# ssttuu/go-pbrt

Hardware: AMD Instinct MI355X
Metric: Mpaths/s (samples×pixels/s) at 1920×1080, 64 spp; 1/2/4/8-GPU scaling + HBM GB/s vs roofline (higher is better)
Workload: dtype f64

## Files before the change

### go-pbrt_amd/csrc/k_chain.h

```cpp
#pragma once
#pragma clang fp contract(off)

#include "render_common.h"

namespace pbrtk {

template <bool kX>
__device__ __forceinline__ uint32_t ring_d(const Cursor& c, const SpecSampler& ss, uint32_t d) {
    if (!kX || c.rri < 0 || d == kBadExactD || c.rrn == 0) return d;
    return kRrFlag | (d == kBadSpecD ? kRrTailBad : d);
}

__device__ __forceinline__ int uni(int v) { return __builtin_amdgcn_readfirstlane(v); }
__device__ __forceinline__ uint32_t uni(uint32_t v) { return (uint32_t)__builtin_amdgcn_readfirstlane((int)v); }
__device__ __forceinline__ float uni(float v) { return __int_as_float(__builtin_amdgcn_readfirstlane(__float_as_int(v))); }
__device__ __forceinline__ uint64_t uni(uint64_t v) {
    return (uint64_t)uni((uint32_t)(v >> 32)) << 32 | uni((uint32_t)v);
}
__device__ __forceinline__ int64_t uni(int64_t v) { return (int64_t)uni((uint64_t)v); }
__device__ __forceinline__ CiGroup uni(const CiGroup& s) {
    CiGroup u;
    u.S = uni(s.S);
    u.pi = uni(s.pi);
    u.npx = uni(s.npx);
    u.A = uni(s.A);
    u.head = uni(s.head);
    u.nxt = uni(s.nxt);
    u.kh = uni(s.kh);
    u.phase = uni(s.phase);
    u.reissue = uni(s.reissue);
    u.rb0 = uni(s.rb0);
    u.rb1 = uni(s.rb1);
    u.nb = uni(s.nb);
    u.nnx = uni(s.nnx);
    u.nps = uni(s.nps);
    u.dcnt = uni(s.dcnt);
    u.dsum = uni(s.dsum);
    u.dsq = uni(s.dsq);
    return u;
}

template <int kW, int kDepth, bool kX, int kEu, bool kSpWin, bool kMulti>
__global__ __launch_bounds__(kWave * kW) __attribute__((amdgpu_waves_per_eu(kEu > 0 ? kEu : kDepth < 0 ? PBRT_CI_MESH_EU_WAVES : kX ? PBRT_CI_X_EU_WAVES : PBRT_CI_EU_WAVES, 8))) void k_chain_ci(
    DevScene sc, RenderParams rp, ChainLayout lay, const PcgJump* __restrict__ jump, WaveBufs wb, int64_t slot_base,
    int64_t nslots_batch, int lanes_per_tile, int ring_size, Counters* __restrict__ ctr,
    const uint32_t* __restrict__ order, uint32_t* __restrict__ ticks, int cstride, uint32_t* __restrict__ prog) {
    extern __shared__ __attribute__((aligned(16))) unsigned char lds[];
    const uint64_t t_begin = wall_clock64();
    if (prog && threadIdx.x == 0) __hip_atomic_fetch_add(&prog[0], 1u, __ATOMIC_RELAXED, __HIP_MEMORY_SCOPE_AGENT);
    const uint32_t cs = cstride == 1 ? 1u : 2u;
    constexpr int kT = kWave * kW;
    __shared__ uint16_t stack_lds[kDepth > 0 ? kDepth * kT : 1];
#ifdef PBRT_CI_DENSE_WALK
    __shared__ __attribute__((aligned(16))) unsigned char dense_lds[kDepth > 0 ? 16 : kW * kDenseScratch];
#endif
    __shared__ CiGroup gs[kCiMaxGroups];
    __shared__ uint64_t sh_state;
    __shared__ uint32_t sh_draws;
    __shared__ int sh_act;
    __shared__ int wcnt[kW];
#ifdef PBRT_CI_DIAG
    __shared__ uint32_t dh[64];
#endif
    static_assert(!kMulti || kW == 1, "several tiles per wave: one-wave workgroups only");
    const int tid = threadIdx.x, lane = tid & (kWave - 1), wv = kW > 1 ? uni(tid / kWave) : 0;
    stage_nodes(sc);
    const int L = kMulti ? lanes_per_tile : kT, G = kMulti ? kWave / L : 1;
    const int g = kMulti ? lane / L : 0, gl = kMulti ? lane - g * L : tid;
    const int64_t blk = order ? (int64_t)order[blockIdx.x] : (int64_t)blockIdx.x;
    const uint32_t R = (uint32_t)ring_size;
    const PcgJump& J = *jump;
    double* s1d = lay.s1d >= 0 ? (double*)(lds + lay.s1d) : nullptr;
    uint16_t* other = (uint16_t*)(lds + lay.other);
    uint32_t* vbuf = (uint32_t*)(lds + lay.vbuf);
    constexpr bool kNps = kW > 1 && !kX;
    const bool nps_on = kNps && rp.ci_nps != 0 && cstride == 1;
    constexpr uint32_t kNpsMinStats = 16;
    constexpr bool kStats = !kX && (kW > 1 || kDepth < 0);
    const float zcap = nps_on ? 3.0f : rp.ci_scap >= 0 ? 0.1f * (float)rp.ci_scap : kDepth < 0 ? 1.5f : 0.0f;
    auto ring_of = [&](int64_t pix) -> RingEnt* {
        return (RingEnt*)(lds + lay.ring) + (size_t)(nps_on ? (int)(pix & 1) : g) * R;
    };
    auto rpar = [&](int64_t pix) -> int { return nps_on ? (int)(pix & 1) : 0; };
    ChainCache* pcs = (ChainCache*)(lds + lay.pcs);
    uint16_t* stack = stack_lds + tid;
    const int n = rp.spp, ndims = rp.ndims;
#ifndef PBRT_CI_TAILCAP
#define PBRT_CI_TAILCAP 1
#endif
    const uint32_t dmax = (uint32_t)(camera_draws(ndims) + 8 * (rp.max_depth + 1) + 8);
    const pbrt_camera_desc& cam = *sc.camera;
    const unsigned long long gmask = !kMulti || L >= 64 ? ~0ULL : (((1ULL << (L & 63)) - 1ULL) << (g * L));
    const int64_t bs = blk * G + g;
    const uint64_t inc = pcg_inc_of((uint64_t)tile_of_slot(rp, slot_base + (bs < nslots_batch ? bs : 0)));
#ifdef PBRT_CI_DIAG
    unsigned long long steps = 0, busy = 0;
    unsigned long long ph[8] = {0, 0, 0, 0, 0, 0, 0, 0};
    long long tprev = clock64();
    auto mark = [&](int k) {
        long long now = clock64();
        ph[k] += (unsigned long long)(now - tprev);
        tprev = now;
    };
    if (tid < 64) dh[tid] = 0;
#define CI_DIAG(x) x
#else
    auto mark = [](int) {};
#define CI_DIAG(x)
#endif
    if (tid < G) {
        const int64_t b = blk * G + tid;
        CiGroup& s = gs[tid];
        s.pi = 0;
        s.kh = 1;
        s.A = s.head = s.nxt = 0;
        s.rb0 = s.rb1 = 0;
        s.nb = s.nnx = 0;
        s.nps = 0;
        s.dcnt = 0;
        s.dsum = s.dsq = 0.0f;
        s.reissue = 0;
        if (b < nslots_batch) {
            int64_t x0, y0, x1, y1;
            tile_bounds(rp, tile_of_slot(rp, slot_base + b), x0, y0, x1, y1);
            Pcg seed;
            pcg_seed(seed, (uint64_t)tile_of_slot(rp, slot_base + b));
            s.S = seed.state;
            s.npx = (x1 - x0) * (y1 - y0);
            s.phase = s.npx > 0 ? 0 : 2;
            wb.tile_npx[b] = 0;
        } else {
            s.S = 0;
            s.npx = 0;
            s.phase = 2;
        }
    }
    __syncthreads();

    uint32_t cancel_poll = 0;
    uint64_t last_host_poll = t_begin;
    uint32_t off = kNoOff;
    int opi_r = -1;
#ifdef PBRT_CI_LDS_STATE
    constexpr bool kLdsState = true;
#else
    constexpr bool kLdsState = kX;
#endif
    __shared__ Spec xs_beta[kLdsState ? kT : 1];
    __shared__ double xs_eta[kLdsState ? kT : 1];
    constexpr bool kStIssue = !kMulti;
    __shared__ uint64_t xs_st0[kLdsState && !kStIssue ? kT : 1];
    uint64_t st0_r = 0;
    Spec beta_r = spec(1);
    double eta_r = 1.0;
    uint64_t& st0 = [&]() -> uint64_t& { if constexpr (kLdsState && !kStIssue) return xs_st0[tid]; else return st0_r; }();
    Spec& beta = [&]() -> Spec& { if constexpr (kLdsState) return xs_beta[tid]; else return beta_r; }();
    double& eta_scale = [&]() -> double& { if constexpr (kLdsState) return xs_eta[tid]; else return eta_r; }();
    st0 = 0;
    beta = spec(1);
    eta_scale = 1.0;
    bool tracing = false;
    Cursor c;
    c.rri = -1;
    c.rrn = 0;
    c.rng.state = 0;
    c.rng.inc = inc;
    c.draws = 0;
    c.cur1d = c.cur2d = 0;
    c.k = -1;
    c.kdep = 0;
    int bounces = 1;
    Ray ray;
    ray.o = ray.d = V3{0, 0, 0};
    ray.tmax = kInf;
    ray.time = 0;

    for (;;) {
        for (int q = 0; q < G; q++) {
            while (gs[q].phase == 0) {
                const int64_t bq = blk * G + q;
                const int64_t tile = tile_of_slot(rp, slot_base + bq);
                const uint64_t incq = pcg_inc_of((uint64_t)tile);
                const int64_t pi = gs[q].pi;
                const int64_t rec = bq * wb.ppt + pi;
                int64_t x0, y0, x1, y1;
                tile_bounds(rp, tile, x0, y0, x1, y1);
                const int64_t px = x0 + pi % (x1 - x0), py = y0 + pi / (x1 - x0);
                double* gs1d = wb.s1d + rec * wb.s1d_stride;
                double* sp = s1d ? s1d : gs1d;
                const uint64_t S1 = start_pixel_wave<kSpWin>(rp, J, gs[q].S, incq, sp, other, vbuf, &sh_state, &sh_draws);
                if (s1d)
                    for (int idx = tid; idx < ndims * n; idx += kT) gs1d[idx] = s1d[idx];
                const double time_u = sp[1 < n ? 1 : 0];
                __syncthreads();
                const bool spec_ran = nps_on && gs[q].nps != 0;
                if (!spec_ran) {
                    RingEnt* rq = nps_on ? ring_of(pi) : (RingEnt*)(lds + lay.ring) + (size_t)q * R;
                    for (uint32_t i = (uint32_t)tid; i < R; i += kT) rq[i].tag = kNoOff;
                }
                PixelRec& pr = wb.prec[rec];
                const int hit0 = pr.hit, panic0 = pr.panic0;
                if (tid == 0) {
                    if (prog)
                        __hip_atomic_fetch_add(&prog[2], 1u, __ATOMIC_RELAXED, __HIP_MEMORY_SCOPE_AGENT);
                    const uint64_t now = wall_clock64();
                    const bool host = now - last_host_poll >= 100000;
                    if (host) last_host_poll = now;
                    if (cancel_requested(sc, host))
                        for (int q2 = 0; q2 < G; q2++) gs[q2].phase = 2;
                }
                if (tid == 0 && gs[q].phase == 0) {
                    if (hit0)
                        pr.si.time = camera_ray(cam, (double)px, (double)py, time_u, V2{0.0, 0.0}).time;
                    ChainCache& pq = pcs[2 * q + rpar(pi)];
                    pq.si = pr.si;
                    pq.b = pr.b;
                    if constexpr (kX) pq.x = pr.x;
                    pq.wo = pr.wo;
                    pq.hit = hit0;
                    CiGroup& s = gs[q];
                    s.S = S1;
                    s.A += sh_draws;
                    s.head = s.A;
                    s.nxt = (spec_ran && s.A >= s.nb) ? max(s.nnx, s.A) : s.A;
                    if (!spec_ran) {
                        if (rpar(pi)) s.rb1 = s.A;
                        else s.rb0 = s.A;
                    }
                    s.nps = 0;
                    s.kh = 1;
                    s.reissue = 0;
                    wb.tile_npx[bq] = (int32_t)(pi + 1);
                    if (panic0) {
                        s.phase = 2;
                    } else if (hit0) {
                        s.phase = 1;
                    } else {
                        if (ndims < 2) {
                            s.S = pcg_advance(J, S1, incq, (uint64_t)(n - 1) * camera_draws(ndims));
                            s.A += (uint32_t)(n - 1) * camera_draws(ndims);
                        }
                        s.pi = pi + 1;
                        s.phase = s.pi < s.npx ? 0 : 2;
                    }
                }
                __syncthreads();
            }
        }
        mark(0);
        bool any_chain = false;
        for (int q = 0; q < G; q++) any_chain |= gs[q].phase == 1;
        if (!any_chain) break;
        CI_DIAG(steps++;)

        CiGroup sg;
        if constexpr (kMulti) sg = gs[g];
        else sg = uni(gs[0]);
        const int64_t rec = bs * wb.ppt + sg.pi;
        const SpecSampler ss{wb.s1d + rec * wb.s1d_stride, n, ndims,
                             kX && wb.rrb ? wb.rrb + bs * kCiMaxRing : nullptr};
        {
            const bool idle = sg.phase == 1 && off == kNoOff;
            const unsigned long long m = __ballot(idle) & gmask;
            int nidle = __popcll(m);
            int rank;
            if constexpr (kMulti) rank = __popcll(m & ((1ULL << lane) - 1ULL));
            else rank = (int)__builtin_amdgcn_mbcnt_hi((uint32_t)(m >> 32), __builtin_amdgcn_mbcnt_lo((uint32_t)m, 0u));
            if (kW > 1) {
                if (lane == 0) wcnt[wv] = nidle;
                __syncthreads();
                int before = 0, tot = 0;
                for (int w = 0; w < kW; w++) {
                    const int cw = wcnt[w];
                    before += w < wv ? cw : 0;
                    tot += cw;
                }
                rank += before;
                nidle = tot;
            }
            const int re = (sg.reissue && nidle > 0) ? 1 : 0;
            const uint32_t nx0 = sg.nxt;
            const int avail = nx0 < sg.head + R ? (int)((sg.head + R - nx0 + cs - 1) / cs) : 0;
#if PBRT_CI_TAILCAP
            const uint32_t tail = sg.head + (uint32_t)(n - 1 - sg.kh) * dmax;
            const int capn = nx0 <= tail ? (int)((tail - nx0) / cs) + 1 : 0;
            int nspec = min(min(nidle - re, avail), capn);
            if (kStats && zcap > 0.0f && sg.dcnt >= kNpsMinStats) {
                const float rem = (float)(n - 1 - sg.kh);
                const float mu = sg.dsum / (float)sg.dcnt;
                const float sd = sqrtf(fmaxf(0.0f, sg.dsq / (float)sg.dcnt - mu * mu));
                const uint32_t scap = sg.head + (uint32_t)(rem * mu + zcap * sd * sqrtf(rem));
                nspec = min(nspec, nx0 <= scap ? (int)((scap - nx0) / cs) + 1 : 0);
            }
#else
            const int nspec = min(nidle - re, avail);
#endif
            int nspec1 = 0;
            if (kNps && sg.phase == 1 && sg.nps) {
                const int avail1 = sg.nnx < sg.nb + R ? (int)(sg.nb + R - sg.nnx) : 0;
                nspec1 = max(0, min(nidle - re - max(nspec, 0), avail1));
            }
            uint32_t o = kNoOff;
            bool exact = false;
            int opix = (int)sg.pi;
            if (idle) {
                if (re && rank == 0) {
                    o = sg.head;
                    exact = true;
                } else {
                    rank -= re;
                    if (rank < nspec) {
                        o = nx0 + cs * (uint32_t)rank;
                    } else if (kNps && rank - nspec < nspec1) {
                        o = sg.nnx + (uint32_t)(rank - nspec);
                        opix = (int)sg.pi + 1;
                    }
                }
            }
            if (gl == 0 && sg.phase == 1) {
                gs[g].nxt = nx0 + cs * (uint32_t)max(nspec, 0);
                if (kNps) gs[g].nnx = sg.nnx + (uint32_t)nspec1;
                CI_DIAG(ph[5] += (unsigned long long)(max(nspec, 0) + nspec1 + re);)
                CI_DIAG(ph[7] += (unsigned long long)nspec1;)
                if (re) gs[g].reissue = 0;
            }
            if (o != kNoOff) {
                off = o;
                if (kNps) opi_r = opix;
                RingEnt& e = ring_of(opix)[(off - (rpar(opix) ? sg.rb1 : sg.rb0)) & (R - 1u)];
                if constexpr (kStIssue) {
                    const uint64_t st = pcg_advance(J, sg.S, inc, (uint64_t)(o - sg.A));
                    e.st = st;
                    c.rng.state = st;
                } else {
                    st0 = pcg_advance(J, sg.S, inc, (uint64_t)(o - sg.A));
                    c.rng.state = st0;
                }
                c.draws = 0;
                c_camera(c, ndims);
                c.k = exact ? sg.kh : -1;
                c.kdep = 0;
                if constexpr (kX) {
                    c.rri = (!exact && ss.rrb) ? (int)((off - sg.rb0) & (R - 1u)) : -1;
                    c.rrn = 0;
                }
                beta = spec(1);
                eta_scale = 1.0;
                bounces = 1;
                const ChainCache& pc = pcs[2 * g + rpar(opix)];
                const int r = traj_scatter<kX>(sc, pc.si, pc.b, pc.x, pc.wo, c, ss, beta, eta_scale, bounces, ray,
                                               rp.max_depth, rp.rr_threshold);
                tracing = r == 0;
                if (r != 0) {
                    if constexpr (!kStIssue) e.st = st0;
                    e.d = ring_d<kX>(c, ss, r == 1 ? c.draws : (c.k >= 0 ? kBadExactD : kBadSpecD));
                    e.tag = off;
                    off = kNoOff;
                }
            }
        }
        const int64_t opi = kNps ? (int64_t)opi_r : sg.pi;
        mark(1);
        CI_DIAG(const unsigned long long tbusy = __ballot(tracing); if (lane == 0) busy += (unsigned long long)__popcll(tbusy);)
#ifdef PBRT_CI_DENSE_WALK
        const bool dense = kDepth == 0 && sc.dense_ok && sc.use_lds_nodes;
        int panic = 0, best = -1;
        V3 ph{0, 0, 0};
        if (dense) bvh_walk_dense(sc, ray, tracing, panic, best, ph, dense_lds + (size_t)wv * kDenseScratch);
        if (tracing) {
            if (!dense) bvh_walk<false, kT, PBRT_CHAIN_LB, (kDepth < 0)>(sc, ray, stack, panic, best, ph);
#else
        if (tracing) {
            int panic = 0, best;
            V3 ph;
            bvh_walk<false, kT, PBRT_CHAIN_LB, (kDepth < 0)>(sc, ray, stack, panic, best, ph);
#endif
            mark(2);
            uint32_t d = kNoOff;
            if (panic) {
                d = c.k >= 0 ? kBadExactD : kBadSpecD;
            } else if (best < 0) {
                d = c.draws;
            } else {
                SI si;
                prim_si(sc, best, ray, ph, si);
                BSDF b;
                BSDFX x;
                if ((kX ? compute_bsdf_x(sc, si, b, x) : compute_bsdf(sc, si, b)) < 0) {
                    d = c.k >= 0 ? kBadExactD : kBadSpecD;
                } else {
                    const int r = traj_scatter<kX>(sc, si, b, x, ray.d, c, ss, beta, eta_scale, bounces, ray,
                                                   rp.max_depth, rp.rr_threshold);
                    if (r == 1) d = c.draws;
                    else if (r == 2) d = c.k >= 0 ? kBadExactD : kBadSpecD;
                }
            }
            if (d != kNoOff) {
                RingEnt& e = ring_of(opi)[(off - (rpar(opi) ? sg.rb1 : sg.rb0)) & (R - 1u)];
                if constexpr (!kStIssue) e.st = st0;
                e.d = ring_d<kX>(c, ss, d);
                e.tag = off;
                off = kNoOff;
                tracing = false;
            }
        }
        mark(3);
        __syncthreads();
        if (gl == 0 && sg.phase == 1) {
            CiGroup s = gs[g];
            if ((++cancel_poll & 127u) == 0) {
                const uint64_t now = wall_clock64();
                const bool host = now - last_host_poll >= 100000;
                if (host) last_host_poll = now;
                if (cancel_requested(sc, host)) s.phase = 2;
            }
            RingEnt* rcur = ring_of(s.pi);
            const uint32_t rbase = rpar(s.pi) ? s.rb1 : s.rb0;
            for (; s.phase == 1;) {
                RingEnt& e = rcur[(s.head - rbase) & (R - 1u)];
                if (e.tag != s.head) break;
                uint32_t d = e.d;
                if (kX && d < kBadExactD && (d & kRrFlag)) {
                    const RrBranches& b = ss.rrb[(s.head - rbase) & (R - 1u)];
                    d = (d & kRrTailBad) == kRrTailBad ? kBadSpecD : (d & kRrTailBad);
                    for (uint32_t i = 0; i < b.n; i++) {
                        const uint32_t cd = b.cd[i];
                        if (ss.s1d[(int)(cd & 0xFFu) * n + s.kh] < b.q[i]) {
                            d = cd >> 8;
                            break;
                        }
                    }
                }
                if (d == kBadSpecD) {
                    e.tag = kNoOff;
                    s.reissue = 1;
                    break;
                }
                wb.memb[rec * n + s.kh] = e.st;
                if (d == kBadExactD) {
                    wb.prec[rec].nvalid = s.kh + 1;
                    s.phase = 2;
                    break;
                }
                CI_DIAG(atomicAdd(&dh[min(d / 2u, 63u)], 1u);)
                CI_DIAG(if (d > dmax) ph[6]++;)
                CI_DIAG(if (d & 1u) atomicAdd(&ctr->odd_d, 1ull);)
                if (kStats) {
                    s.dcnt++;
                    s.dsum += (float)d;
                    s.dsq += (float)d * (float)d;
                }
                s.kh++;
                s.head += d;
                if (s.kh >= n) {
                    s.S = pcg_advance(J, s.S, inc, (uint64_t)(s.head - s.A));
                    s.A = s.head;
                    s.pi++;
                    s.phase = s.pi < s.npx ? 0 : 2;
                    break;
                }
            }
            if (s.nxt < s.head || (cs == 2u && ((s.nxt ^ s.head) & 1u))) s.nxt = s.head;
            int act = 0;
            const int left = n - s.kh;
            const bool stats = s.dcnt >= kNpsMinStats;
            if (nps_on && s.phase == 1 && !s.nps && (left == 1 || (stats && left <= rp.ci_nps)) &&
                s.pi + 1 < s.npx) {
                const PixelRec& pn = wb.prec[rec + 1];
                if (pn.hit && !pn.panic0) {
                    float lo = 0.0f;
                    if (left > 1) {
                        const float mu = s.dsum / (float)s.dcnt;
                        const float sd = sqrtf(fmaxf(0.0f, s.dsq / (float)s.dcnt - mu * mu));
                        lo = fmaxf(0.0f, (float)left * mu - 3.0f * sd * sqrtf((float)left));
                    }
                    s.nps = 1;
                    s.nb = s.head + (uint32_t)lo + (uint32_t)rp.sp_events;
                    s.nnx = s.nb;
                    if (rpar(s.pi + 1)) s.rb1 = s.nb;
                    else s.rb0 = s.nb;
                    act = 1;
                }
            }
            if (kNps) sh_act = act;
            CiGroup& gw = gs[g];
            gw.S = s.S;
            gw.A = s.A;
            gw.pi = s.pi;
            gw.head = s.head;
            gw.nxt = s.nxt;
            gw.kh = s.kh;
            gw.phase = s.phase;
            gw.reissue = s.reissue;
            if (kStats) {
                gw.dcnt = s.dcnt;
                gw.dsum = s.dsum;
                gw.dsq = s.dsq;
            }
            if (kNps) {
                gw.nps = s.nps;
                gw.nb = s.nb;
                gw.nnx = s.nnx;
                gw.rb0 = s.rb0;
                gw.rb1 = s.rb1;
            }
        }
        if (kNps && tid == 0 && !(gl == 0 && sg.phase == 1)) sh_act = 0;
        __syncthreads();
        if (kNps && sh_act) {
            const CiGroup s3 = uni(gs[0]);
            RingEnt* rn = ring_of(s3.pi + 1);
            for (uint32_t i = (uint32_t)tid; i < R; i += kT) rn[i].tag = kNoOff;
            if (tid == 0) {
                const PixelRec& pn = wb.prec[rec + 1];
                ChainCache& pc = pcs[2 * g + rpar(s3.pi + 1)];
                pc.si = pn.si;
                pc.b = pn.b;
                pc.wo = pn.wo;
                pc.hit = pn.hit;
            }
        }
        if (off != kNoOff) {
            const CiGroup s2 = gs[g];
            bool keep = false;
            if ((!kNps || opi == s2.pi) && s2.phase == 1)
                keep = !(off < s2.head || (cs == 2u && ((off ^ s2.head) & 1u)) ||
                         (PBRT_CI_TAILCAP && off > s2.head + (uint32_t)(n - 1 - s2.kh) * dmax));
            else if (kNps && opi == s2.pi && s2.phase == 0)
                keep = s2.nps != 0;
            else if (kNps && opi == s2.pi + 1 && s2.phase == 1)
                keep = s2.nps != 0;
            if (!keep) {
                off = kNoOff;
                tracing = false;
            }
        }
        mark(4);
    }
#ifdef PBRT_CI_DIAG
    __syncthreads();
    if (tid < 64 && dh[tid]) atomicAdd(&ctr->dhist[tid], (unsigned long long)dh[tid]);
    if (tid == 0) {
        atomicAdd(&ctr->windows, steps);
        for (int k = 0; k < 8; k++) atomicAdd(&ctr->phase[k], ph[k]);
        atomicAdd(&ctr->nps_issued, ph[7]);
    }
    if (lane == 0) atomicAdd(&ctr->busy, busy);
#endif
#undef CI_DIAG
    if (prog) {
        __threadfence();
        __syncthreads();
    }
    if (tid == 0) {
        if (prog && G == 1 && bs < nslots_batch) {
            const uint32_t pos = __hip_atomic_fetch_add(&prog[1], 1u, __ATOMIC_RELAXED, __HIP_MEMORY_SCOPE_AGENT);
            __hip_atomic_store(&prog[kProgHead + pos], (uint32_t)bs, __ATOMIC_RELEASE, __HIP_MEMORY_SCOPE_AGENT);
        }
        if (ticks && G == 1 && bs < nslots_batch) {
            const uint64_t t_end = wall_clock64();
            ticks[bs] = (uint32_t)min(t_end - t_begin, (uint64_t)0xFFFFFFFFu);
#ifdef PBRT_CI_DIAG
            ticks[nslots_batch + bs] = (uint32_t)t_begin;
            ticks[2 * nslots_batch + bs] = (uint32_t)t_end;
#endif
        }
    }
}

}
```

Measured before the change: 371.2.

## Reorder chain loop so fresh and hit scatters share one traj_scatter call site

Restructures the chain-issue loop into traverse, scatter and walk_drop lambdas. For depth-limited, non-window kernels it rotates the loop so traversal and ring drain run at the top of the iteration, and a single scatter call handles both freshly issued chains and BVH hits. This removes the duplicated traj_scatter call site, which is meant to cut code size, register pressure and divergent execution of two scatter paths. The rotation changes the order of phases relative to the barriers and hoists sg, rec and ss out of the loop, which risks subtle state-ordering bugs.

```diff
diff --git a/go-pbrt_amd/csrc/k_chain.h b/go-pbrt_amd/csrc/k_chain.h
--- a/go-pbrt_amd/csrc/k_chain.h
+++ b/go-pbrt_amd/csrc/k_chain.h
@@ -95,11 +95,11 @@
     const uint64_t inc = pcg_inc_of((uint64_t)tile_of_slot(rp, slot_base + (bs < nslots_batch ? bs : 0)));
 #ifdef PBRT_CI_DIAG
     unsigned long long steps = 0, busy = 0;
-    unsigned long long ph[8] = {0, 0, 0, 0, 0, 0, 0, 0};
+    unsigned long long ph_cyc[8] = {0, 0, 0, 0, 0, 0, 0, 0};
     long long tprev = clock64();
     auto mark = [&](int k) {
         long long now = clock64();
-        ph[k] += (unsigned long long)(now - tprev);
+        ph_cyc[k] += (unsigned long long)(now - tprev);
         tprev = now;
     };
     if (tid < 64) dh[tid] = 0;
@@ -175,7 +175,216 @@
     ray.tmax = kInf;
     ray.time = 0;
 
+    CiGroup sg;
+    if constexpr (kMulti) sg = gs[g];
+    else sg = uni(gs[0]);
+    int64_t rec = bs * wb.ppt + sg.pi;
+    SpecSampler ss{wb.s1d + rec * wb.s1d_stride, n, ndims, kX && wb.rrb ? wb.rrb + bs * kCiMaxRing : nullptr};
+
+    constexpr bool kOneScatter = kDepth >= 0 && !kSpWin;
+    using Both = std::integral_constant<int, 0>;
+    using Fresh = std::integral_constant<int, 1>;
+    using Hits = std::integral_constant<int, 2>;
+    int best = -1;
+    V3 ph{0, 0, 0};
+    auto traverse = [&]() __attribute__((always_inline)) {
+        const int64_t opi = kNps ? (int64_t)opi_r : sg.pi;
+        best = -1;
+        int panic = 0;
+#ifdef PBRT_CI_DENSE_WALK
+        const bool dense = kDepth == 0 && sc.dense_ok && sc.use_lds_nodes;
+        if (dense) bvh_walk_dense(sc, ray, tracing, panic, best, ph, dense_lds + (size_t)wv * kDenseScratch);
+        if (tracing) {
+            if (!dense) bvh_walk<false, kT, PBRT_CHAIN_LB, (kDepth < 0)>(sc, ray, stack, panic, best, ph);
+#else
+        if (tracing) {
+            bvh_walk<false, kT, PBRT_CHAIN_LB, (kDepth < 0)>(sc, ray, stack, panic, best, ph);
+#endif
+            if (panic || best < 0) {
+                RingEnt& e = ring_of(opi)[(off - (rpar(opi) ? sg.rb1 : sg.rb0)) & (R - 1u)];
+                if constexpr (!kStIssue) e.st = st0;
+                e.d = ring_d<kX>(c, ss, panic ? (c.k >= 0 ? kBadExactD : kBadSpecD) : c.draws);
+                e.tag = off;
+                off = kNoOff;
+                tracing = false;
+            }
+        }
+    };
+    auto scatter = [&](auto which, bool fresh) __attribute__((always_inline)) {
+        constexpr int kWhich = decltype(which)::value;
+        const bool first = kWhich == Fresh::value ? true : kWhich == Hits::value ? false : fresh;
+        if (kWhich == Fresh::value ? fresh : kWhich == Hits::value ? tracing : (fresh || tracing)) {
+            const int64_t spi = kNps ? (int64_t)opi_r : sg.pi;
+            SI si;
+            BSDF b;
+            BSDFX x;
+            V3 wo = ray.d;
+            bool ok = true;
+            if (first) {
+                const ChainCache& pc = pcs[2 * g + rpar(spi)];
+                si = pc.si;
+                b = pc.b;
+                if constexpr (kX) x = pc.x;
+                wo = pc.wo;
+            } else {
+                prim_si(sc, best, ray, ph, si);
+                ok = (kX ? compute_bsdf_x(sc, si, b, x) : compute_bsdf(sc, si, b)) >= 0;
+            }
+            const int r = !ok ? 2
+                              : traj_scatter<kX>(sc, si, b, x, wo, c, ss, beta, eta_scale, bounces, ray, rp.max_depth,
+                                                 rp.rr_threshold);
+            tracing = r == 0;
+            if (r != 0) {
+                RingEnt& e = ring_of(spi)[(off - (rpar(spi) ? sg.rb1 : sg.rb0)) & (R - 1u)];
+                if constexpr (!kStIssue) e.st = st0;
+                e.d = ring_d<kX>(c, ss, r == 1 ? c.draws : (c.k >= 0 ? kBadExactD : kBadSpecD));
+                e.tag = off;
+                off = kNoOff;
+            }
+        }
+    };
+    auto walk_drop = [&]() __attribute__((always_inline)) {
+        const int64_t opi = kNps ? (int64_t)opi_r : sg.pi;
+        __syncthreads();
+        if (gl == 0 && sg.phase == 1) {
+            CiGroup s = gs[g];
+            if ((++cancel_poll & 127u) == 0) {
+                const uint64_t now = wall_clock64();
+                const bool host = now - last_host_poll >= 100000;
+                if (host) last_host_poll = now;
+                if (cancel_requested(sc, host)) s.phase = 2;
+            }
+            RingEnt* rcur = ring_of(s.pi);
+            const uint32_t rbase = rpar(s.pi) ? s.rb1 : s.rb0;
+            for (; s.phase == 1;) {
+                RingEnt& e = rcur[(s.head - rbase) & (R - 1u)];
+                if (e.tag != s.head) break;
+                uint32_t d = e.d;
+                if (kX && d < kBadExactD && (d & kRrFlag)) {
+                    const RrBranches& b = ss.rrb[(s.head - rbase) & (R - 1u)];
+                    d = (d & kRrTailBad) == kRrTailBad ? kBadSpecD : (d & kRrTailBad);
+                    for (uint32_t i = 0; i < b.n; i++) {
+                        const uint32_t cd = b.cd[i];
+                        if (ss.s1d[(int)(cd & 0xFFu) * n + s.kh] < b.q[i]) {
+                            d = cd >> 8;
+                            break;
+                        }
+                    }
+                }
+                if (d == kBadSpecD) {
+                    e.tag = kNoOff;
+                    s.reissue = 1;
+                    break;
+                }
+                wb.memb[rec * n + s.kh] = e.st;
+                if (d == kBadExactD) {
+                    wb.prec[rec].nvalid = s.kh + 1;
+                    s.phase = 2;
+                    break;
+                }
+                CI_DIAG(atomicAdd(&dh[min(d / 2u, 63u)], 1u);)
+                CI_DIAG(if (d > dmax) ph_cyc[6]++;)
+                CI_DIAG(if (d & 1u) atomicAdd(&ctr->odd_d, 1ull);)
+                if (kStats) {
+                    s.dcnt++;
+                    s.dsum += (float)d;
+                    s.dsq += (float)d * (float)d;
+                }
+                s.kh++;
+                s.head += d;
+                if (s.kh >= n) {
+                    s.S = pcg_advance(J, s.S, inc, (uint64_t)(s.head - s.A));
+                    s.A = s.head;
+                    s.pi++;
+                    s.phase = s.pi < s.npx ? 0 : 2;
+                    break;
+                }
+            }
+            if (s.nxt < s.head || (cs == 2u && ((s.nxt ^ s.head) & 1u))) s.nxt = s.head;
+            int act = 0;
+            const int left = n - s.kh;
+            const bool stats = s.dcnt >= kNpsMinStats;
+            if (nps_on && s.phase == 1 && !s.nps && (left == 1 || (stats && left <= rp.ci_nps)) &&
+                s.pi + 1 < s.npx) {
+                const PixelRec& pn = wb.prec[rec + 1];
+                if (pn.hit && !pn.panic0) {
+                    float lo = 0.0f;
+                    if (left > 1) {
+                        const float mu = s.dsum / (float)s.dcnt;
+                        const float sd = sqrtf(fmaxf(0.0f, s.dsq / (float)s.dcnt - mu * mu));
+                        lo = fmaxf(0.0f, (float)left * mu - 3.0f * sd * sqrtf((float)left));
+                    }
+                    s.nps = 1;
+                    s.nb = s.head + (uint32_t)lo + (uint32_t)rp.sp_events;
+                    s.nnx = s.nb;
+                    if (rpar(s.pi + 1)) s.rb1 = s.nb;
+                    else s.rb0 = s.nb;
+                    act = 1;
+                }
+            }
+            if (kNps) sh_act = act;
+            CiGroup& gw = gs[g];
+            gw.S = s.S;
+            gw.A = s.A;
+            gw.pi = s.pi;
+            gw.head = s.head;
+            gw.nxt = s.nxt;
+            gw.kh = s.kh;
+            gw.phase = s.phase;
+            gw.reissue = s.reissue;
+            if (kStats) {
+                gw.dcnt = s.dcnt;
+                gw.dsum = s.dsum;
+                gw.dsq = s.dsq;
+            }
+            if (kNps) {
+                gw.nps = s.nps;
+                gw.nb = s.nb;
+                gw.nnx = s.nnx;
+                gw.rb0 = s.rb0;
+                gw.rb1 = s.rb1;
+            }
+        }
+        if (kNps && tid == 0 && !(gl == 0 && sg.phase == 1)) sh_act = 0;
+        __syncthreads();
+        if (kNps && sh_act) {
+            const CiGroup s3 = uni(gs[0]);
+            RingEnt* rn = ring_of(s3.pi + 1);
+            for (uint32_t i = (uint32_t)tid; i < R; i += kT) rn[i].tag = kNoOff;
+            if (tid == 0) {
+                const PixelRec& pn = wb.prec[rec + 1];
+                ChainCache& pc = pcs[2 * g + rpar(s3.pi + 1)];
+                pc.si = pn.si;
+                pc.b = pn.b;
+                pc.wo = pn.wo;
+                pc.hit = pn.hit;
+            }
+        }
+        if (off != kNoOff) {
+            const CiGroup s2 = gs[g];
+            bool keep = false;
+            if ((!kNps || opi == s2.pi) && s2.phase == 1)
+                keep = !(off < s2.head || (cs == 2u && ((off ^ s2.head) & 1u)) ||
+                         (PBRT_CI_TAILCAP && off > s2.head + (uint32_t)(n - 1 - s2.kh) * dmax));
+            else if (kNps && opi == s2.pi && s2.phase == 0)
+                keep = s2.nps != 0;
+            else if (kNps && opi == s2.pi + 1 && s2.phase == 1)
+                keep = s2.nps != 0;
+            if (!keep) {
+                off = kNoOff;
+                tracing = false;
+            }
+        }
+    };
+
     for (;;) {
+        if constexpr (kOneScatter) {
+            CI_DIAG(const unsigned long long tbusy = __ballot(tracing); if (lane == 0) busy += (unsigned long long)__popcll(tbusy);)
+            traverse();
+            mark(2);
+            walk_drop();
+            mark(4);
+        }
         for (int q = 0; q < G; q++) {
             while (gs[q].phase == 0) {
                 const int64_t bq = blk * G + q;
@@ -188,7 +397,8 @@
                 const int64_t px = x0 + pi % (x1 - x0), py = y0 + pi / (x1 - x0);
                 double* gs1d = wb.s1d + rec * wb.s1d_stride;
                 double* sp = s1d ? s1d : gs1d;
-                const uint64_t S1 = start_pixel_wave<kSpWin>(rp, J, gs[q].S, incq, sp, other, vbuf, &sh_state, &sh_draws);
+                uint64_t S1;
+                [[clang::always_inline]] S1 = start_pixel_wave<kSpWin>(rp, J, gs[q].S, incq, sp, other, vbuf, &sh_state, &sh_draws);
                 if (s1d)
                     for (int idx = tid; idx < ndims * n; idx += kT) gs1d[idx] = s1d[idx];
                 const double time_u = sp[1 < n ? 1 : 0];
@@ -253,12 +463,11 @@
         if (!any_chain) break;
         CI_DIAG(steps++;)
 
-        CiGroup sg;
         if constexpr (kMulti) sg = gs[g];
         else sg = uni(gs[0]);
-        const int64_t rec = bs * wb.ppt + sg.pi;
-        const SpecSampler ss{wb.s1d + rec * wb.s1d_stride, n, ndims,
-                             kX && wb.rrb ? wb.rrb + bs * kCiMaxRing : nullptr};
+        rec = bs * wb.ppt + sg.pi;
+        ss.s1d = wb.s1d + rec * wb.s1d_stride;
+        bool fresh = false;
         {
             const bool idle = sg.phase == 1 && off == kNoOff;
             const unsigned long long m = __ballot(idle) & gmask;
@@ -320,8 +529,8 @@
             if (gl == 0 && sg.phase == 1) {
                 gs[g].nxt = nx0 + cs * (uint32_t)max(nspec, 0);
                 if (kNps) gs[g].nnx = sg.nnx + (uint32_t)nspec1;
-                CI_DIAG(ph[5] += (unsigned long long)(max(nspec, 0) + nspec1 + re);)
-                CI_DIAG(ph[7] += (unsigned long long)nspec1;)
+                CI_DIAG(ph_cyc[5] += (unsigned long long)(max(nspec, 0) + nspec1 + re);)
+                CI_DIAG(ph_cyc[7] += (unsigned long long)nspec1;)
                 if (re) gs[g].reissue = 0;
             }
             if (o != kNoOff) {
@@ -347,203 +556,32 @@
                 beta = spec(1);
                 eta_scale = 1.0;
                 bounces = 1;
-                const ChainCache& pc = pcs[2 * g + rpar(opix)];
-                const int r = traj_scatter<kX>(sc, pc.si, pc.b, pc.x, pc.wo, c, ss, beta, eta_scale, bounces, ray,
-                                               rp.max_depth, rp.rr_threshold);
-                tracing = r == 0;
-                if (r != 0) {
-                    if constexpr (!kStIssue) e.st = st0;
-                    e.d = ring_d<kX>(c, ss, r == 1 ? c.draws : (c.k >= 0 ? kBadExactD : kBadSpecD));
-                    e.tag = off;
-                    off = kNoOff;
-                }
-            }
-        }
-        const int64_t opi = kNps ? (int64_t)opi_r : sg.pi;
-        mark(1);
-        CI_DIAG(const unsigned long long tbusy = __ballot(tracing); if (lane == 0) busy += (unsigned long long)__popcll(tbusy);)
-#ifdef PBRT_CI_DENSE_WALK
-        const bool dense = kDepth == 0 && sc.dense_ok && sc.use_lds_nodes;
-        int panic = 0, best = -1;
-        V3 ph{0, 0, 0};
-        if (dense) bvh_walk_dense(sc, ray, tracing, panic, best, ph, dense_lds + (size_t)wv * kDenseScratch);
-        if (tracing) {
-            if (!dense) bvh_walk<false, kT, PBRT_CHAIN_LB, (kDepth < 0)>(sc, ray, stack, panic, best, ph);
-#else
-        if (tracing) {
-            int panic = 0, best;
-            V3 ph;
-            bvh_walk<false, kT, PBRT_CHAIN_LB, (kDepth < 0)>(sc, ray, stack, panic, best, ph);
-#endif
+                fresh = true;
+            }
+        }
+        if constexpr (kOneScatter) {
+            mark(1);
+            scatter(Both{}, fresh);
+            mark(3);
+        } else {
+            scatter(Fresh{}, fresh);
+            mark(1);
+            CI_DIAG(const unsigned long long tbusy = __ballot(tracing); if (lane == 0) busy += (unsigned long long)__popcll(tbusy);)
+            traverse();
             mark(2);
-            uint32_t d = kNoOff;
-            if (panic) {
-                d = c.k >= 0 ? kBadExactD : kBadSpecD;
-            } else if (best < 0) {
-                d = c.draws;
-            } else {
-                SI si;
-                prim_si(sc, best, ray, ph, si);
-                BSDF b;
-                BSDFX x;
-                if ((kX ? compute_bsdf_x(sc, si, b, x) : compute_bsdf(sc, si, b)) < 0) {
-                    d = c.k >= 0 ? kBadExactD : kBadSpecD;
-                } else {
-                    const int r = traj_scatter<kX>(sc, si, b, x, ray.d, c, ss, beta, eta_scale, bounces, ray,
-                                                   rp.max_depth, rp.rr_threshold);
-                    if (r == 1) d = c.draws;
-                    else if (r == 2) d = c.k >= 0 ? kBadExactD : kBadSpecD;
-                }
-            }
-            if (d != kNoOff) {
-                RingEnt& e = ring_of(opi)[(off - (rpar(opi) ? sg.rb1 : sg.rb0)) & (R - 1u)];
-                if constexpr (!kStIssue) e.st = st0;
-                e.d = ring_d<kX>(c, ss, d);
-                e.tag = off;
-                off = kNoOff;
-                tracing = false;
-            }
-        }
-        mark(3);
-        __syncthreads();
-        if (gl == 0 && sg.phase == 1) {
-            CiGroup s = gs[g];
-            if ((++cancel_poll & 127u) == 0) {
-                const uint64_t now = wall_clock64();
-                const bool host = now - last_host_poll >= 100000;
-                if (host) last_host_poll = now;
-                if (cancel_requested(sc, host)) s.phase = 2;
-            }
-            RingEnt* rcur = ring_of(s.pi);
-            const uint32_t rbase = rpar(s.pi) ? s.rb1 : s.rb0;
-            for (; s.phase == 1;) {
-                RingEnt& e = rcur[(s.head - rbase) & (R - 1u)];
-                if (e.tag != s.head) break;
-                uint32_t d = e.d;
-                if (kX && d < kBadExactD && (d & kRrFlag)) {
-                    const RrBranches& b = ss.rrb[(s.head - rbase) & (R - 1u)];
-                    d = (d & kRrTailBad) == kRrTailBad ? kBadSpecD : (d & kRrTailBad);
-                    for (uint32_t i = 0; i < b.n; i++) {
-                        const uint32_t cd = b.cd[i];
-                        if (ss.s1d[(int)(cd & 0xFFu) * n + s.kh] < b.q[i]) {
-                            d = cd >> 8;
-                            break;
-                        }
-                    }
-                }
-                if (d == kBadSpecD) {
-                    e.tag = kNoOff;
-                    s.reissue = 1;
-                    break;
-                }
-                wb.memb[rec * n + s.kh] = e.st;
-                if (d == kBadExactD) {
-                    wb.prec[rec].nvalid = s.kh + 1;
-                    s.phase = 2;
-                    break;
-                }
-                CI_DIAG(atomicAdd(&dh[min(d / 2u, 63u)], 1u);)
-                CI_DIAG(if (d > dmax) ph[6]++;)
-                CI_DIAG(if (d & 1u) atomicAdd(&ctr->odd_d, 1ull);)
-                if (kStats) {
-                    s.dcnt++;
-                    s.dsum += (float)d;
-                    s.dsq += (float)d * (float)d;
-                }
-                s.kh++;
-                s.head += d;
-                if (s.kh >= n) {
-                    s.S = pcg_advance(J, s.S, inc, (uint64_t)(s.head - s.A));
-                    s.A = s.head;
-                    s.pi++;
-                    s.phase = s.pi < s.npx ? 0 : 2;
-                    break;
-                }
-            }
-            if (s.nxt < s.head || (cs == 2u && ((s.nxt ^ s.head) & 1u))) s.nxt = s.head;
-            int act = 0;
-            const int left = n - s.kh;
-            const bool stats = s.dcnt >= kNpsMinStats;
-            if (nps_on && s.phase == 1 && !s.nps && (left == 1 || (stats && left <= rp.ci_nps)) &&
-                s.pi + 1 < s.npx) {
-                const PixelRec& pn = wb.prec[rec + 1];
-                if (pn.hit && !pn.panic0) {
-                    float lo = 0.0f;
-                    if (left > 1) {
-                        const float mu = s.dsum / (float)s.dcnt;
-                        const float sd = sqrtf(fmaxf(0.0f, s.dsq / (float)s.dcnt - mu * mu));
-                        lo = fmaxf(0.0f, (float)left * mu - 3.0f * sd * sqrtf((float)left));
-                    }
-                    s.nps = 1;
-                    s.nb = s.head + (uint32_t)lo + (uint32_t)rp.sp_events;
-                    s.nnx = s.nb;
-                    if (rpar(s.pi + 1)) s.rb1 = s.nb;
-                    else s.rb0 = s.nb;
-                    act = 1;
-                }
-            }
-            if (kNps) sh_act = act;
-            CiGroup& gw = gs[g];
-            gw.S = s.S;
-            gw.A = s.A;
-            gw.pi = s.pi;
-            gw.head = s.head;
-            gw.nxt = s.nxt;
-            gw.kh = s.kh;
-            gw.phase = s.phase;
-            gw.reissue = s.reissue;
-            if (kStats) {
-                gw.dcnt = s.dcnt;
-                gw.dsum = s.dsum;
-                gw.dsq = s.dsq;
-            }
-            if (kNps) {
-                gw.nps = s.nps;
-                gw.nb = s.nb;
-                gw.nnx = s.nnx;
-                gw.rb0 = s.rb0;
-                gw.rb1 = s.rb1;
-            }
-        }
-        if (kNps && tid == 0 && !(gl == 0 && sg.phase == 1)) sh_act = 0;
-        __syncthreads();
-        if (kNps && sh_act) {
-            const CiGroup s3 = uni(gs[0]);
-            RingEnt* rn = ring_of(s3.pi + 1);
-            for (uint32_t i = (uint32_t)tid; i < R; i += kT) rn[i].tag = kNoOff;
-            if (tid == 0) {
-                const PixelRec& pn = wb.prec[rec + 1];
-                ChainCache& pc = pcs[2 * g + rpar(s3.pi + 1)];
-                pc.si = pn.si;
-                pc.b = pn.b;
-                pc.wo = pn.wo;
-                pc.hit = pn.hit;
-            }
-        }
-        if (off != kNoOff) {
-            const CiGroup s2 = gs[g];
-            bool keep = false;
-            if ((!kNps || opi == s2.pi) && s2.phase == 1)
-                keep = !(off < s2.head || (cs == 2u && ((off ^ s2.head) & 1u)) ||
-                         (PBRT_CI_TAILCAP && off > s2.head + (uint32_t)(n - 1 - s2.kh) * dmax));
-            else if (kNps && opi == s2.pi && s2.phase == 0)
-                keep = s2.nps != 0;
-            else if (kNps && opi == s2.pi + 1 && s2.phase == 1)
-                keep = s2.nps != 0;
-            if (!keep) {
-                off = kNoOff;
-                tracing = false;
-            }
-        }
-        mark(4);
+            scatter(Hits{}, false);
+            mark(3);
+            walk_drop();
+            mark(4);
+        }
     }
 #ifdef PBRT_CI_DIAG
     __syncthreads();
     if (tid < 64 && dh[tid]) atomicAdd(&ctr->dhist[tid], (unsigned long long)dh[tid]);
     if (tid == 0) {
         atomicAdd(&ctr->windows, steps);
-        for (int k = 0; k < 8; k++) atomicAdd(&ctr->phase[k], ph[k]);
-        atomicAdd(&ctr->nps_issued, ph[7]);
+        for (int k = 0; k < 8; k++) atomicAdd(&ctr->phase[k], ph_cyc[k]);
+        atomicAdd(&ctr->nps_issued, ph_cyc[7]);
     }
     if (lane == 0) atomicAdd(&ctr->busy, busy);
 #endif
```

Result: faster. 379.4 (median of 6 runs) (+2.2%).
